# haowenz/FEM

Measured on AMD Instinct MI355X. Metric: mapped Mreads/s (100 bp, e=3) at 1/2/4/8 MI355X + achieved HBM GB/s vs roofline, higher is better.
Workload: dtype u32/u64 integer + 32-bit Myers bit-vectors

## Files before the change

fem_amd/csrc/fem_hip.hip:

```cpp
#include "../../include/fem_hip.h"

#include <hip/hip_runtime.h>
#include <rccl/rccl.h>
#include <sched.h>
#if defined(__x86_64__)
#include <immintrin.h>
#endif

#include <algorithm>
#include <cctype>
#include <cstdio>
#include <cstdlib>
#include <cstring>
#include <condition_variable>
#include <functional>
#include <atomic>
#include <chrono>
#include <mutex>
#include <string>
#include <thread>
#include <vector>

#include "fem_index_build.hip.h"
#include "fem_pack.h"
#include "fem_kernels.hip.h"
#include "fem_seed_fast.hip.h"
#include "fem_seed_join.hip.h"
#include "fem_tail.hip.h"
#include "fem_bgzf.hip.h"

namespace {

#ifndef FEM_SLOTS
#define FEM_SLOTS 4
#endif
constexpr int kSlots = FEM_SLOTS;
constexpr uint32_t kMaxReadLen = 1024;
constexpr size_t kFrontPad = 16;
constexpr uint32_t kXcapSmall = 512, kFcap = 128, kCcap = 128;

constexpr int kTimedKernels = 15;
struct TimedLaunch {
  int kernel;
  hipEvent_t start, stop;
  bool counts = true;
};
constexpr int kMaxParts = 4;

struct Slot {
  hipStream_t stream = nullptr;
  uint8_t *d_bases_alloc = nullptr;
  uint8_t *bases() const { return d_bases_alloc + 16; }
  size_t bases_cap = 0;
  uint64_t *d_off = nullptr;
  size_t off_cap = 0;
  uint64_t n_reads = 0;
  uint64_t n_bases = 0;
  uint32_t max_len = 0;
  bool staged = false;
  char *h_bases = nullptr;
  size_t h_bases_cap = 0;
  uint64_t *h_off = nullptr;
  size_t h_off_cap = 0;
  uint64_t acq_reads = 0, acq_bases = 0;
  char *h_quals = nullptr, *h_names = nullptr;
  uint64_t *h_name_off = nullptr;
  size_t h_quals_cap = 0, h_names_cap = 0, h_name_off_cap = 0;
  uint8_t *d_quals = nullptr, *d_names = nullptr;
  uint64_t *d_name_off = nullptr;
  size_t d_quals_cap = 0, d_names_cap = 0, d_name_off_cap = 0;
  bool text_staged = false;
  bool host_quals = false;
  const uint64_t *qual_at = nullptr;
  hipStream_t text_stream = nullptr;
  hipStream_t out_stream = nullptr;
  hipEvent_t ev_text_staged = nullptr;
  hipEvent_t ev_text_order = nullptr;
  bool have_text_order = false;
  uint8_t *d_packed = nullptr;
  size_t packed_cap = 0;
  uint32_t *d_exc_bits = nullptr;
  size_t exc_bits_cap = 0;
  uint32_t packed_bpr = 0;
  bool prefetch_results = false, staged_by_copy = false;
  uint64_t prefetched_reads2 = 0, prefetched_cand = 0, last_n_cand = 0;
  uint64_t h2d_bytes = 0;
  bool sent_packed = false;
  int parts = 1;
  uint32_t part_begin[kMaxParts + 1] = {0, 0, 0, 0, 0};
  hipEvent_t ev_part[kMaxParts] = {nullptr, nullptr, nullptr, nullptr}, ev_sel[kMaxParts] = {nullptr, nullptr, nullptr, nullptr};
  hipEvent_t ev_zeroed = nullptr;
  hipEvent_t ev_results = nullptr, ev_home = nullptr;
  uint64_t *d_cand = nullptr;
  uint32_t *d_meta = nullptr;
  uint8_t *d_ed = nullptr;
  int16_t *d_end = nullptr;
  uint32_t cand_cap = 0;
  uint32_t *d_begin = nullptr, *d_count = nullptr, *d_nmap = nullptr;
  size_t per_read_cap = 0;
  uint8_t *d_ctl = nullptr;
  uint8_t *h_ctl = nullptr;
  uint64_t *d_arena = nullptr;
  uint64_t arena_cap = 0;
  uint32_t *d_slow = nullptr;
  uint32_t slow_cap = 0;
  uint2 *d_sel = nullptr, *d_sel_hdr = nullptr;
  size_t sel_cap = 0, sel_hdr_cap = 0;
  uint32_t *h_begin = nullptr, *h_count = nullptr;
  size_t h_per_read_cap = 0;
  uint64_t *h_cand = nullptr;
  uint8_t *h_ed = nullptr;
  int16_t *h_end = nullptr;
// ... 93 lines not shown
  std::condition_variable cv_, done_;
  std::vector<std::thread> threads_;
  const std::function<void(unsigned)> *work_ = nullptr;
  unsigned n_ = 0, pending_ = 0;
  uint64_t epoch_ = 0;
  bool stop_ = false;
};
}

struct fem_dev {
  femt::TextGate text_gate;
  femz::Bgzf *bgzf = nullptr;
  uint8_t *d_zin = nullptr;
  size_t d_zin_cap = 0;
  hipStream_t z_stream = nullptr;
  std::recursive_mutex mu;
  int device = 0;
  StagePool *stage_pool = nullptr;
  uint8_t *d_ref_names = nullptr;
  uint32_t *d_ref_name_off = nullptr;
  int n_cu = 256;
  std::string err;
  uint32_t *d_lookup = nullptr;
  uint64_t n_lookup = 0;
  uint64_t *d_occ = nullptr;
  uint64_t n_occ = 0;
  int32_t k = 0, step = 0;
  uint64_t fast_occ_key = ~0ull;
  int fast_occ_blocks = 0;
  uint32_t *d_summary = nullptr;
  uint32_t *d_occ32 = nullptr, *d_goff = nullptr, *d_blkseq = nullptr;
  uint32_t list_shift = 0;
  bool no_strided = false;
  uint32_t *d_freq11 = nullptr;
  uint32_t n_banks = 1, bank_first[5] = {0, 0, 0, 0, 0};
  uint32_t *d_bank_lo = nullptr;
  uint64_t bank_limit = 0;
  uint32_t bank_seqs = 0;
  int select_occ_blocks = 0, join_occ_blocks = 0;
  uint64_t select_occ_key = ~0ull, join_occ_key = ~0ull;
  uint8_t *d_planes = nullptr;
  uint8_t *d_ref_raw = nullptr;
  uint64_t ref_bytes = 0;
  uint64_t *d_seq_off = nullptr;
  uint32_t *d_seq_len = nullptr;
  uint32_t n_seq = 0;
  std::vector<uint64_t> seq_off;
  std::vector<uint32_t> seq_len;
  Slot slot[kSlots];
  bool timing = false;
  int verify_blocks_per_cu = 0;
  double t_ms[kTimedKernels] = {};
  uint64_t t_n[kTimedKernels] = {};
  bool force_generic = false;
  bool force_hash = false;
  bool force_dense = false;
  bool no_dense = false;
  bool tiny_buffers = false;
  std::vector<hipEvent_t> event_pool;
  hipEvent_t ev_kernels_done = nullptr;
  bool have_kernels_done = false;
  hipEvent_t ev_select_done = nullptr;
  bool have_select_done = false;
  bool no_overlap = false;
  hipEvent_t ev_h2d_done = nullptr;
  bool have_h2d_done = false;
  hipStream_t side_stream = nullptr;
  bool no_parts = false;
  int max_parts = 2;
  bool timeline = false, have_epoch = false;
  hipEvent_t ev_epoch = nullptr;
};

namespace {

bool testing_switch(const char *name) {
  const char *t = getenv("FEM_TESTING");
  if (!(t && t[0] == '1')) return false;
  const char *v = getenv(name);
  return v && v[0] == '1';
}

int fail(fem_dev *h, int rc, const std::string &msg) {
  if (h) {
// ... 547 lines not shown
    *wpb_out = wpb, *lds_out = lds_bytes;
    *grid_out = (uint32_t)std::max<uint64_t>(1, std::min<uint64_t>(blocks_wanted, blocks_resident * 4));
  };
  if (sp.lay.wave_bytes > 64u * 1024u) return fail(h, FEM_ERR_UNSUPPORTED, "read too long for the device path");

  auto timed = [&](int id, hipStream_t st, auto &&launch, bool counts = true) -> int {
    TimedLaunch t{id, nullptr, nullptr, counts};
    if (h->timing) {
      t.start = get_event(h), t.stop = get_event(h);
      HIP_TRY(h, hipEventRecord(t.start, st));
    }
    launch();
    HIP_TRY(h, hipGetLastError());
    if (h->timing) {
      HIP_TRY(h, hipEventRecord(t.stop, st));
      s.pending.push_back(t);
    }
    return FEM_OK;
  };

  if (s.n_reads) {
    int rc;
    const bool split_dense = use_fast && h->d_occ32 && h->d_freq11;
    const bool overlap = split_dense && !h->no_overlap;
    if (!overlap && h->have_kernels_done) HIP_TRY(h, hipStreamWaitEvent(s.stream, h->ev_kernels_done, 0));
    femk::VerifyParams vp{};
    vp.bases = s.bases(), vp.read_off = s.d_off;
    vp.planes = h->d_planes, vp.seq_off = h->d_seq_off;
    vp.cand = s.d_cand, vp.cand_meta = s.d_meta;
    vp.ctr = d_ctr, vp.cand_cap = s.cand_cap, vp.e = p.e;
    vp.ed = s.d_ed, vp.end = s.d_end;
    vp.n_map = s.d_nmap, vp.stats = d_stats;
    HIP_TRY(h, hipMemsetAsync(s.d_nmap, 0, (size_t)s.n_reads * sizeof(uint32_t), s.stream));
    if (h->verify_blocks_per_cu == 0) {
      int nb = 0;
      if (hipOccupancyMaxActiveBlocksPerMultiprocessor(&nb, femk::verify_kernel, 256, 0) != hipSuccess || nb <= 0) nb = 4;
      h->verify_blocks_per_cu = nb;
    }
    const uint32_t vgrid = (uint32_t)h->n_cu * (uint32_t)h->verify_blocks_per_cu;
    if (split_dense) {
      const uint32_t max_len = std::max<uint32_t>(s.max_len, (uint32_t)p.k);
      const bool banked = h->n_banks > 1;
      const size_t want_sel = (size_t)s.n_reads * 6u * (size_t)R * h->n_banks;
      if ((rc = dev_realloc(h, &s.d_sel, &s.sel_cap, want_sel))) return rc;
      if ((rc = dev_realloc(h, &s.d_sel_hdr, &s.sel_hdr_cap, (size_t)s.n_reads))) return rc;
      femk::SeedParams fp = sp;
      fp.occ32 = h->d_occ32, fp.list_shift = h->list_shift, fp.goff = h->d_goff, fp.blkseq = h->d_blkseq;
      fp.freq11 = h->d_freq11, fp.sel = s.d_sel, fp.sel_hdr = s.d_sel_hdr;
      fp.n_banks = h->n_banks, fp.bank_lo = h->d_bank_lo, fp.n_buckets = (uint32_t)(h->n_lookup - 1);
      fp.blk_stride = (femk::kDenseRemap >> femk::kDenseBlkShift) + 1u;
      for (uint32_t b = 0; b <= femk::kDenseMaxBanks; ++b) fp.bank_first[b] = h->bank_first[b];
      uint32_t select_lds = 0, select_threads = 256;
      fp.lay = make_layout_select(p, max_len);
      if (fp.lay.wave_bytes > 64u * 1024u) return fail(h, FEM_ERR_UNSUPPORTED, "read too long for the device path");
      const femk::SeedLayout lay_select = fp.lay;
      femk::SeedLayout lay_join = make_layout_join(p, banked, !banked && h->list_shift != 0);
      const uint32_t wpb_s = std::min<uint32_t>(4u, std::max<uint32_t>(1u, (64u * 1024u) / lay_select.wave_bytes));
      const uint32_t wpb_j = std::min<uint32_t>(4u, std::max<uint32_t>(1u, (60u * 1024u) / lay_join.wave_bytes));
      lay_join.picked = wpb_j * lay_join.wave_bytes;
      const uint32_t lds_j = wpb_j * lay_join.wave_bytes + 64u * 8u;
      const int which = banked ? 1 : h->list_shift ? 2 : 0;
      uint64_t per_cu_s, per_cu_j;
      {
        const uint32_t lds_bytes = wpb_s * lay_select.wave_bytes;
        const uint64_t key = ((uint64_t)banked << 48) | ((uint64_t)R << 40) | lds_bytes;
        if (h->select_occ_key != key) h->select_occ_key = key, h->select_occ_blocks = select_blocks_per_cu(R, banked, (int)(64u * wpb_s), lds_bytes);
        per_cu_s = h->select_occ_blocks > 0 ? (uint64_t)h->select_occ_blocks : std::max<uint64_t>(1, 160u * 1024u / lds_bytes);
        if (overlap) per_cu_s = 1;
        select_lds = lds_bytes, select_threads = 64u * wpb_s;
      }
      {
        const uint64_t key = ((uint64_t)which << 48) | ((uint64_t)R << 40) | lds_j;
// ... 56 lines not shown
        if (h->fast_occ_key != key) h->fast_occ_key = key, h->fast_occ_blocks = fast_blocks_per_cu((int)R, hash, (int)(64u * wpb), lds_bytes);
        static const uint64_t mult = testing_switch("FEM_TESTING") && getenv("FEM_GRID_MULT") ? (uint64_t)std::max(1, atoi(getenv("FEM_GRID_MULT"))) : 1;
        const uint64_t per_cu = h->fast_occ_blocks > 0 ? (uint64_t)h->fast_occ_blocks : std::max<uint64_t>(1, 160u * 1024u / lds_bytes);
        const uint64_t wanted = (s.n_reads + (uint64_t)femk::kReadBlock * wpb - 1) / ((uint64_t)femk::kReadBlock * wpb);
        grid = (uint32_t)std::max<uint64_t>(1, std::min<uint64_t>(wanted, (uint64_t)h->n_cu * per_cu * mult));
      }
      auto launch_range = [&](uint32_t lo, uint32_t hi) {
        femk::SeedParams q = fp;
        q.read_begin = lo, q.n_reads = hi;
        dim3 g(grid), b(64u * wpb);
        switch (R) {
          case 1: launch_fast<1>(hash, g, b, lds_bytes, s.stream, q); break;
          case 2: launch_fast<2>(hash, g, b, lds_bytes, s.stream, q); break;
          case 3: launch_fast<3>(hash, g, b, lds_bytes, s.stream, q); break;
          case 4: launch_fast<4>(hash, g, b, lds_bytes, s.stream, q); break;
          case 5: launch_fast<5>(hash, g, b, lds_bytes, s.stream, q); break;
          case 6: launch_fast<6>(hash, g, b, lds_bytes, s.stream, q); break;
          case 7: launch_fast<7>(hash, g, b, lds_bytes, s.stream, q); break;
          case 8: launch_fast<8>(hash, g, b, lds_bytes, s.stream, q); break;
          case 9: launch_fast<9>(hash, g, b, lds_bytes, s.stream, q); break;
          default: launch_fast<10>(hash, g, b, lds_bytes, s.stream, q); break;
        }
      };
      rc = timed(0, s.stream, [&] { launch_range(0, (uint32_t)s.n_reads); });
      if (rc) return rc;
      sp.work_queue = s.d_slow;
    }
    {
      uint32_t wpb, lds_bytes, grid;
      shape(sp.lay, &wpb, &lds_bytes, &grid);
      rc = timed(2, s.stream, [&] { hipLaunchKernelGGL(femk::seed_filter_kernel, dim3(grid), dim3(64u * wpb), lds_bytes, s.stream, sp); });
      if (rc) return rc;
    }
    rc = timed(1, s.stream, [&] { hipLaunchKernelGGL(femk::verify_kernel, dim3(vgrid), dim3(256), 0, s.stream, vp); });
    if (rc) return rc;
    s.packed_enqueued = false, s.packed_home = 0, s.packed_per_read_home = false;
    if (s.want_packed && split_dense && (rc = enqueue_pack(h, s, true, false))) return rc;
    HIP_TRY(h, hipEventRecord(h->ev_kernels_done, s.stream));
    h->have_kernels_done = true;
    if (s.want_packed && (rc = enqueue_pack(h, s, !split_dense, true))) return rc;
  } else {
    s.packed_enqueued = false, s.packed_home = 0, s.packed_per_read_home = false;
  }
  HIP_TRY(h, hipMemcpyAsync(s.h_ctl, s.d_ctl, kCtlBytes, hipMemcpyDeviceToHost, s.stream));
  s.prefetched_reads2 = 0, s.prefetched_cand = 0;
  static const bool no_prefetch = testing_switch("FEM_NO_PREFETCH");
  if (s.prefetch_results && !s.want_packed && s.staged_by_copy && !no_prefetch) {
    hipStream_t st = d2h_begin(h, s);
    {
      Span span(h, s, 21, st);
      const size_t n2 = (size_t)s.n_reads * 2;
      if (n2 && s.h_begin && n2 <= s.h_per_read_cap) {
        HIP_TRY(h, hipMemcpyAsync(s.h_begin, s.d_begin, n2 * sizeof(uint32_t), hipMemcpyDeviceToHost, st));
        HIP_TRY(h, hipMemcpyAsync(s.h_count, s.d_count, n2 * sizeof(uint32_t), hipMemcpyDeviceToHost, st));
        s.prefetched_reads2 = n2;
      }
      const size_t guess = std::min<size_t>({(size_t)(s.last_n_cand + s.last_n_cand / 32 + 1024), s.h_cand_cap, (size_t)s.cand_cap});
      if (s.last_n_cand && s.h_cand && guess) {
        HIP_TRY(h, hipMemcpyAsync(s.h_cand, s.d_cand, guess * sizeof(uint64_t), hipMemcpyDeviceToHost, st));
        HIP_TRY(h, hipMemcpyAsync(s.h_ed, s.d_ed, guess * sizeof(uint8_t), hipMemcpyDeviceToHost, st));
        HIP_TRY(h, hipMemcpyAsync(s.h_end, s.d_end, guess * sizeof(int16_t), hipMemcpyDeviceToHost, st));
        s.prefetched_cand = guess;
      }
    }
    int rc2 = d2h_end(h, s, st);
    if (rc2) return rc2;
  }
// ... 126 lines not shown

struct CommSet {
  std::vector<int> devs;
  std::vector<ncclComm_t> comms;
  std::vector<uint64_t *> bufs;
};
std::mutex g_comm_mu;
CommSet *g_comm = nullptr;
void destroy_comm_set() {
  if (!g_comm) return;
  for (size_t i = 0; i < g_comm->devs.size(); ++i) {
    (void)hipSetDevice(g_comm->devs[i]);
    if (g_comm->bufs[i]) (void)hipFree(g_comm->bufs[i]);
    if (g_comm->comms[i]) ncclCommDestroy(g_comm->comms[i]);
  }
  delete g_comm;
  g_comm = nullptr;
}

int check_slot(fem_dev *h, int slot) {
  if (!h) return FEM_ERR_INVALID;
  if (slot < 0 || slot >= kSlots) return fail(h, FEM_ERR_INVALID, "slot out of range");
  return FEM_OK;
}


using fempack::pack_bases;

int enqueue_packed(fem_dev *h, Slot &s, uint64_t n, uint32_t len, uint64_t n_exc) {
  const uint32_t bpr = fempack::bytes_per_read(len);
  const uint64_t code_bytes = fempack::code_bytes(n, len), n_bases = n * (uint64_t)len;
  const uint64_t total = code_bytes + n_exc * 5u;
  int rc;
  if ((rc = dev_realloc(h, &s.d_packed, &s.packed_cap, (size_t)total + 64))) return rc;
  if ((rc = dev_realloc(h, &s.d_bases_alloc, &s.bases_cap, kFrontPad + (size_t)n_bases + 64))) return rc;
  if ((rc = dev_realloc(h, &s.d_off, &s.off_cap, (size_t)n + 1))) return rc;
  if ((rc = dev_realloc(h, &s.d_exc_bits, &s.exc_bits_cap, (size_t)n / 32 + 2))) return rc;
  s.parts = 1;
  if (!h->no_parts && !h->no_overlap && n_exc == 0 && n >= 2 * kPartMinReads && device_idle(h))
    s.parts = (int)std::min<uint64_t>((uint64_t)h->max_parts, n / kPartMinReads);
  for (int q = 0; q <= s.parts; ++q) s.part_begin[q] = q == s.parts ? (uint32_t)n : (uint32_t)((n * q / s.parts) & ~63ull);
  HIP_TRY(h, hipMemsetAsync(s.d_exc_bits, 0, ((size_t)n / 32 + 1) * sizeof(uint32_t), s.stream));
  hipLaunchKernelGGL(femk::uniform_offsets_kernel, dim3((uint32_t)std::min<uint64_t>((n + 256) / 256, (uint64_t)h->n_cu * 8u)), dim3(256), 0,
                     s.stream, s.d_off, n, len);
  if ((rc = h2d_begin(h, s))) return rc;
  for (int q = 0; q < s.parts; ++q) {
    const uint64_t r0 = s.part_begin[q], r1 = s.part_begin[q + 1];
    const uint64_t b0 = r0 * bpr, b1 = q + 1 == s.parts ? total : r1 * bpr;
    Span span(h, s, 20, s.stream);
    if (b1 > b0) HIP_TRY(h, hipMemcpyAsync(s.d_packed + b0, s.h_bases + b0, b1 - b0, hipMemcpyHostToDevice, s.stream));
    if (q + 1 == s.parts && (rc = h2d_end(h, s))) return rc;
    if (r1 > r0) {
      const uint32_t grid = (uint32_t)std::min<uint64_t>(((r1 - r0) * bpr + 255) / 256, (uint64_t)h->n_cu * 16u);
      hipLaunchKernelGGL(femk::unpack_reads_kernel, dim3(grid), dim3(256), 0, s.stream, (const uint8_t *)s.d_packed + b0, r1 - r0, len, bpr,
                         s.bases() + r0 * len);
    }
    if (s.parts > 1) HIP_TRY(h, hipEventRecord(s.ev_part[q], s.stream));
  }
  if (n_exc) {
    const dim3 g((uint32_t)std::min<uint64_t>((n_exc + 255) / 256, (uint64_t)h->n_cu * 4u));
    hipLaunchKernelGGL(femk::scatter_chars_kernel, g, dim3(256), 0, s.stream, (const uint32_t *)(s.d_packed + code_bytes),
                       (const uint8_t *)(s.d_packed + code_bytes + 4u * n_exc), n_exc, s.bases());
    hipLaunchKernelGGL(femk::mark_exception_reads_kernel, g, dim3(256), 0, s.stream, (const uint32_t *)(s.d_packed + code_bytes), n_exc, len,
                       s.d_exc_bits);
  }
  s.packed_bpr = bpr;
  HIP_TRY(h, hipGetLastError());
  s.n_reads = n, s.n_bases = n_bases, s.max_len = len;
  s.staged = true, s.mapped = false, s.synced = false;
  s.h2d_bytes = total, s.sent_packed = true;
  return FEM_OK;
}

unsigned stage_threads(uint64_t n_reads) {
  unsigned want = 12;
  if (const char *e = getenv("FEM_STAGE_THREADS")) want = (unsigned)std::max(1, atoi(e));
  const unsigned hw = std::thread::hardware_concurrency();
  return (unsigned)std::max<uint64_t>(1, std::min<uint64_t>({(uint64_t)(hw ? hw : 1), (uint64_t)want, n_reads / 65536 + 1}));
}

}

extern "C" {

const char *fem_strerror(int rc) {
  switch (rc) {
    case FEM_OK: return "ok";
    case FEM_ERR_INVALID: return "invalid argument";
    case FEM_ERR_HIP: return "HIP runtime error";
    case FEM_ERR_NOMEM: return "out of memory";
    case FEM_ERR_STATE: return "call order violated";
    case FEM_ERR_UNSUPPORTED: return "input not supported by the device path";
    case FEM_ERR_RCCL: return "RCCL error";
    default: return "unknown error";
  }
}
// ... 27 lines not shown
      delete h;
      return FEM_ERR_HIP;
    }
  }
  bool ok_ev = hipEventCreateWithFlags(&h->ev_kernels_done, hipEventDisableTiming) == hipSuccess &&
               hipEventCreateWithFlags(&h->ev_select_done, hipEventDisableTiming) == hipSuccess &&
               hipEventCreateWithFlags(&h->ev_h2d_done, hipEventDisableTiming) == hipSuccess &&
               hipStreamCreateWithFlags(&h->side_stream, hipStreamNonBlocking) == hipSuccess;
  for (int i = 0; ok_ev && i < kSlots; ++i) {
    Slot &sl = h->slot[i];
    ok_ev = hipEventCreateWithFlags(&sl.ev_zeroed, hipEventDisableTiming) == hipSuccess &&
            hipEventCreateWithFlags(&sl.ev_results, hipEventDisableTiming) == hipSuccess &&
            hipEventCreateWithFlags(&sl.ev_home, hipEventDisableTiming) == hipSuccess;
    for (int q = 0; ok_ev && q < kMaxParts; ++q)
      ok_ev = hipEventCreateWithFlags(&sl.ev_part[q], hipEventDisableTiming) == hipSuccess &&
              hipEventCreateWithFlags(&sl.ev_sel[q], hipEventDisableTiming) == hipSuccess;
  }
  if (!ok_ev) {
    (void)fem_dev_close(h);
    return FEM_ERR_HIP;
  }
  if (testing_switch("FEM_TESTING")) {
    h->no_overlap = testing_switch("FEM_NO_OVERLAP");
    h->no_parts = testing_switch("FEM_NO_PARTS");
    if (const char *mp = getenv("FEM_PARTS")) h->max_parts = std::min(kMaxParts, std::max(1, atoi(mp)));
    h->timeline = testing_switch("FEM_TIMELINE");
    if (h->timeline && hipEventCreate(&h->ev_epoch) == hipSuccess && hipEventRecord(h->ev_epoch, h->side_stream) == hipSuccess)
      h->timing = true, h->have_epoch = true;
    h->force_generic = testing_switch("FEM_FORCE_GENERIC");
    h->force_hash = testing_switch("FEM_FORCE_HASH");
    h->force_dense = testing_switch("FEM_FORCE_DENSE");
    h->no_dense = testing_switch("FEM_NO_DENSE");
    h->no_strided = testing_switch("FEM_NO_STRIDED");
    h->tiny_buffers = testing_switch("FEM_TEST_TINY_BUFFERS");
    if (const char *bl = getenv("FEM_TEST_BANK_BASES")) h->bank_limit = strtoull(bl, nullptr, 10);
    if (const char *bs = getenv("FEM_TEST_BANK_SEQS")) h->bank_seqs = (uint32_t)strtoul(bs, nullptr, 10);
  }
  *out = h;
  return FEM_OK;
}

int fem_dev_close(fem_dev *h) {
  if (!h) return FEM_ERR_INVALID;
  {
    std::lock_guard<std::mutex> lock(g_comm_mu);
    if (g_comm && std::find(g_comm->devs.begin(), g_comm->devs.end(), h->device) != g_comm->devs.end()) destroy_comm_set();
  }
  (void)hipSetDevice(h->device);
  (void)hipDeviceSynchronize();
  delete h->stage_pool;
  h->stage_pool = nullptr;
  for (auto &s : h->slot) {
    drain_timing(h, s);
    for (void *p : {(void *)s.d_bases_alloc, (void *)s.d_off, (void *)s.d_cand, (void *)s.d_meta, (void *)s.d_ed,
                    (void *)s.d_end, (void *)s.d_begin, (void *)s.d_count, (void *)s.d_nmap, (void *)s.d_ctl,
                    (void *)s.d_arena, (void *)s.d_slow, (void *)s.d_sel, (void *)s.d_sel_hdr, (void *)s.d_packed, (void *)s.d_exc_bits, (void *)s.d_quals, (void *)s.d_names,
                    (void *)s.d_name_off, (void *)s.d_count8, (void *)s.d_seg, (void *)s.d_pcand, (void *)s.d_ped, (void *)s.d_pend, (void *)s.d_big})
      if (p) (void)hipFree(p);
    for (void *p : {(void *)s.h_ctl, (void *)s.h_begin, (void *)s.h_count, (void *)s.h_cand, (void *)s.h_ed,
                    (void *)s.h_end, (void *)s.h_bases, (void *)s.h_off, (void *)s.h_quals, (void *)s.h_names, (void *)s.h_name_off,
                    (void *)s.h_count8, (void *)s.h_seg, (void *)s.h_pcand, (void *)s.h_ped, (void *)s.h_pend, (void *)s.h_big})
      if (p) (void)hipHostFree(p);
    if (s.stream) (void)hipStreamDestroy(s.stream);
    if (s.text_stream) (void)hipStreamDestroy(s.text_stream);
    if (s.out_stream) (void)hipStreamDestroy(s.out_stream);
    if (s.ev_text_staged) (void)hipEventDestroy(s.ev_text_staged);
    if (s.ev_text_order) (void)hipEventDestroy(s.ev_text_order);
    delete s.tail;
    s.tail = nullptr;
  }
  delete h->bgzf;
  h->bgzf = nullptr;
  if (h->d_zin) (void)hipFree(h->d_zin);
  if (h->z_stream) (void)hipStreamDestroy(h->z_stream);
  if (h->d_ref_names) (void)hipFree(h->d_ref_names);
  if (h->d_ref_name_off) (void)hipFree(h->d_ref_name_off);
  for (hipEvent_t e : h->event_pool) (void)hipEventDestroy(e);
  if (h->ev_kernels_done) (void)hipEventDestroy(h->ev_kernels_done);
  if (h->ev_select_done) (void)hipEventDestroy(h->ev_select_done);
  if (h->ev_h2d_done) (void)hipEventDestroy(h->ev_h2d_done);
  if (h->ev_epoch) (void)hipEventDestroy(h->ev_epoch);
  if (h->side_stream) (void)hipStreamDestroy(h->side_stream);
  for (int i = 0; i < kSlots; ++i) {
    Slot &sl = h->slot[i];
    if (sl.ev_zeroed) (void)hipEventDestroy(sl.ev_zeroed);
    if (sl.ev_results) (void)hipEventDestroy(sl.ev_results);
    if (sl.ev_home) (void)hipEventDestroy(sl.ev_home);
    for (int q = 0; q < kMaxParts; ++q) {
      if (sl.ev_part[q]) (void)hipEventDestroy(sl.ev_part[q]);
// ... 594 lines not shown
  return FEM_OK;
}

static hipStream_t out_stream_of(fem_dev *h, Slot &s) {
  static const bool plain = testing_switch("FEM_NO_OUT_PRIORITY");
  if (plain) return s.stream;
  if (!s.out_stream) {
    int least = 0, greatest = 0;
    if (hipDeviceGetStreamPriorityRange(&least, &greatest) != hipSuccess ||
        hipStreamCreateWithPriority(&s.out_stream, hipStreamNonBlocking, greatest) != hipSuccess)
      s.out_stream = nullptr;
  }
  (void)h;
  return s.out_stream ? s.out_stream : s.stream;
}

int fem_dev_reserve_batch(fem_dev *h, int slot, uint64_t n_reads, uint64_t n_records, uint32_t max_len, const fem_params *p) {
  int rc = check_slot(h, slot);
  if (rc) return rc;
  FEM_LOCK(h);
  if (!params_ok(p)) return fail(h, FEM_ERR_INVALID, "parameters out of range (k 1..16, step 1..16, e 0..7, a 0..2)");
  if (!h->d_lookup) return fail(h, FEM_ERR_STATE, "the index must be uploaded first (what a batch needs depends on it)");
  if (n_reads == 0 || n_reads > 0x7FFFFFF0ull || n_records > 0xFFFFFFF0ull || max_len == 0 || max_len > kMaxReadLen)
    return fail(h, FEM_ERR_INVALID, "batch shape out of range");
  Slot &s = h->slot[slot];
  if (s.mapped && !s.synced) return fail(h, FEM_ERR_STATE, "a batch is in flight in this slot");
  HIP_TRY(h, hipSetDevice(h->device));
  const uint64_t n_was = s.n_reads;
  s.n_reads = n_reads;
  rc = ensure_outputs(h, s);
  s.n_reads = n_was;
  if (rc) return rc;
  const uint64_t n_bases = n_reads * (uint64_t)max_len;
  if ((rc = dev_realloc(h, &s.d_packed, &s.packed_cap, (size_t)fempack::code_bytes(n_reads, max_len) + 64))) return rc;
  if ((rc = dev_realloc(h, &s.d_bases_alloc, &s.bases_cap, kFrontPad + (size_t)n_bases + 64))) return rc;
  if ((rc = dev_realloc(h, &s.d_off, &s.off_cap, (size_t)n_reads + 1))) return rc;
  if ((rc = dev_realloc(h, &s.d_exc_bits, &s.exc_bits_cap, (size_t)n_reads / 32 + 2))) return rc;
  if (h->d_occ32 && h->d_freq11 && p->k == 12 && p->step == 3) {
    const size_t R = (size_t)(p->e + 1 + p->a);
    if ((rc = dev_realloc(h, &s.d_sel, &s.sel_cap, (size_t)n_reads * 6u * R * h->n_banks))) return rc;
    if ((rc = dev_realloc(h, &s.d_sel_hdr, &s.sel_hdr_cap, (size_t)n_reads))) return rc;
  }
  if (!s.tail) s.tail = new (std::nothrow) femt::Tail();
  if (!s.tail) return fail(h, FEM_ERR_NOMEM, "out of host memory");
  std::string err;
  if ((rc = s.tail->reserve((uint32_t)n_reads, (uint32_t)n_records, max_len, p->e, h->tiny_buffers, &err))) return fail(h, rc, err);
  if (!s.text_stream) HIP_TRY(h, hipStreamCreateWithFlags(&s.text_stream, hipStreamNonBlocking));
  HIP_TRY(h, hipMemsetAsync(s.d_sel_hdr ? (void *)s.d_sel_hdr : (void *)s.d_off, 0, 8, s.text_stream));
  HIP_TRY(h, hipStreamSynchronize(s.text_stream));
  HIP_TRY(h, hipMemsetAsync(s.d_off, 0, 8, h->side_stream));
  HIP_TRY(h, hipStreamSynchronize(h->side_stream));
  const size_t probe = 1u << 20;
  if (s.h_bases && s.h_bases_cap >= probe && s.bases_cap >= kFrontPad + probe)
    HIP_TRY(h, hipMemcpyAsync(s.d_bases_alloc + kFrontPad, s.h_bases, probe, hipMemcpyHostToDevice, s.stream));
  if (s.h_quals && s.d_quals && s.h_quals_cap >= probe && s.d_quals_cap >= probe)
    HIP_TRY(h, hipMemcpyAsync(s.d_quals, s.h_quals, probe, hipMemcpyHostToDevice, s.text_stream));
  HIP_TRY(h, hipMemcpyAsync(s.h_ctl, s.d_ctl, kCtlBytes, hipMemcpyDeviceToHost, s.stream));
  HIP_TRY(h, hipStreamSynchronize(s.text_stream));
  HIP_TRY(h, hipStreamSynchronize(s.stream));
  if ((rc = s.tail->warm(out_stream_of(h, s), &err))) return fail(h, rc, err);
  return FEM_OK;
}

static int commit_text(fem_dev *h, int slot, uint64_t n_reads, uint64_t n_name_bytes, bool with_quals) {
  int rc = check_slot(h, slot);
  if (rc) return rc;
  FEM_LOCK(h);
// ... 31 lines not shown
  if (!qual_at) return fail(h, FEM_ERR_INVALID, "null output pointer");
  if (!s.host_quals || !s.qual_at) return fail(h, FEM_ERR_STATE, "the slot's last SAM text was rendered with its qualities (or there is none)");
  *qual_at = s.qual_at;
  if (n_reads) *n_reads = s.n_reads;
  return FEM_OK;
}

static int fetch_sam(fem_dev *h, int slot, fem_batch_sam *out, bool wait);
int fem_dev_fetch_sam(fem_dev *h, int slot, fem_batch_sam *out) { return fetch_sam(h, slot, out, true); }
int fem_dev_fetch_sam_nowait(fem_dev *h, int slot, fem_batch_sam *out) { return fetch_sam(h, slot, out, false); }
int fem_dev_sam_wait(fem_dev *h, int slot) {
  if (!h || slot < 0 || slot >= kSlots) return FEM_ERR_INVALID;
  Slot &s = h->slot[slot];
  if (!s.tail) return FEM_ERR_STATE;
  if (hipSetDevice(h->device) != hipSuccess) return FEM_ERR_HIP;
  return s.tail->wait_text();
}

static int rescue_input(fem_dev *h, const Slot &s, femt::RescueInput *ri) {
  if (!s.rescue) return FEM_OK;
  if ((int64_t)s.max_insert - s.min_insert > 65536)
    return fail(h, FEM_ERR_UNSUPPORTED, "mate rescue searches insert windows of at most 65536 (max_insert - min_insert)");
  ri->max_edits = s.rescue_edits;
  ri->bases = s.bases(), ri->read_off = s.d_off, ri->max_len = s.max_len;
  ri->ref_raw = h->d_ref_raw, ri->ref_bytes = h->ref_bytes + 64, ri->seq_off = h->d_seq_off, ri->seq_len = h->d_seq_len;
  return FEM_OK;
}

static femt::TailInput tail_input(const fem_dev *h, const Slot &s) {
  femt::TailInput in{};
  in.bases = s.bases(), in.read_off = s.d_off, in.n_reads = (uint32_t)s.n_reads, in.max_len = s.max_len;
  in.ref_raw = h->d_ref_raw, in.ref_bytes = h->ref_bytes + 64, in.seq_off = h->d_seq_off;
  in.planes = h->d_planes;
  if (s.sent_packed) in.packed = s.d_packed, in.packed_bpr = s.packed_bpr, in.exc_bits = s.d_exc_bits;
  in.cand = s.d_cand, in.ed = s.d_ed, in.end = s.d_end, in.cand_begin = s.d_begin, in.cand_count = s.d_count;
  in.n_map = s.d_nmap, in.e = s.params.e, in.n_records = s.stats[4];
  return in;
}

struct TailFront {
  femt::TailInput in;
  femt::TailOutput t;
  hipStream_t stream;
  double ms[3], ms_sync, ms_run;
  std::chrono::steady_clock::time_point t_in;
};

static int tail_records(fem_dev *h, int slot, const void *out, bool copy_records, bool device_quals, TailFront *f) {
  f->t_in = std::chrono::steady_clock::now();
  auto since = [&]() { return std::chrono::duration<double, std::milli>(std::chrono::steady_clock::now() - f->t_in).count(); };
  int rc = fem_dev_sync(h, slot);
  if (rc) return rc;
  f->ms_sync = since();
  if (!out) return fail(h, FEM_ERR_INVALID, "null result");
  Slot &s = h->slot[slot];
  const bool text = !copy_records, paired = text && s.paired;
  if (text && !s.text_staged) return fail(h, FEM_ERR_STATE, "qualities and names of this batch were not committed (fem_dev_commit_text_stage)");
  if (device_quals && s.host_quals) return fail(h, FEM_ERR_STATE, "BAM records need the qualities on the device (fem_dev_commit_text_stage, not _names_stage)");
  if (text && !h->d_ref_names) return fail(h, FEM_ERR_STATE, "reference names must be uploaded first (fem_dev_upload_reference_names)");
  s.prefetch_results = false;
  if (!s.tail) s.tail = new (std::nothrow) femt::Tail();
  if (!s.tail) return fail(h, FEM_ERR_NOMEM, "out of host memory");
  f->in = tail_input(h, s);
  if (paired && (s.n_reads & 1)) return fail(h, FEM_ERR_INVALID, "a batch of read pairs holds an even number of reads");
  if (copy_records && s.out_stream) HIP_TRY(h, hipStreamSynchronize(s.out_stream));
  f->stream = copy_records ? s.stream : out_stream_of(h, s);
  std::string err;
// ... 493 lines not shown
```

fem_amd/csrc/fem_kernels.hip.h:

```cpp
#pragma once
#include <hip/hip_runtime.h>
#include <stdint.h>
#include "fem_planes.hip.h"

namespace femk {

constexpr int kWave = 64;
constexpr uint32_t kFlagCandOverflow = 1u;
constexpr uint32_t kFlagArenaOverflow = 2u;
constexpr uint32_t kFlagTooLarge = 4u;
constexpr uint32_t kInvalidMeta = 0xFFFFFFFFu;
constexpr int kMaxR = 10;
constexpr uint32_t kMeta16 = 0x80000000u;
constexpr uint32_t kSlotChunk = 256u;
constexpr uint32_t kFlagQueueOverflow = 8u;
constexpr uint32_t kQueueChunk = 32u;
constexpr uint32_t kInvalidRead = 0xFFFFFFFFu;

struct SeedLayout {
  uint32_t pkw, nkw;
  uint32_t sf;
  uint32_t dp_rows;
  uint32_t dp_bits;
  uint32_t picked;
// ... 1102 lines not shown
          } else {
            if (ln == 0) atomicOr(&p.ctr[1], kFlagTooLarge);
          }
        }
      }
      wave_sync_lds();
      STAMP(prof, 7);
    }
  }
  pad_chunk(p, chunk);
#ifdef FEM_STAMPS
  prof.flush();
#endif
  if (ln == 0) {
    if (pre_sum) atomicAdd(&p.stats[0], pre_sum);
    if (cand_sum) atomicAdd(&p.stats[1], cand_sum);
  }
}

struct VerifyParams {
  const uint8_t *bases;
  const uint64_t *read_off;
  const uint8_t *planes;
  const uint64_t *seq_off;
  const uint64_t *cand;
  const uint32_t *cand_meta;
  const uint32_t *ctr;
  uint32_t cand_cap;
  int32_t e;
  uint8_t *ed;
  int16_t *end;
  uint32_t *n_map;
  unsigned long long *stats;
};

__device__ __forceinline__ uint4 load_u128_unaligned(const uint8_t *p) {
  uint4 w;
  __builtin_memcpy(&w, p, 16);
  return w;
}

__device__ __forceinline__ uint4 plane_window(const uint8_t *planes, int q, uint64_t at) {
  return load_u128_unaligned(plane_addr(planes, q, at));
}
__device__ __forceinline__ uint32_t load_u32_unaligned(const uint8_t *p) {
  uint32_t w;
  __builtin_memcpy(&w, p, 4);
  return w;
}

struct MyersState {
  uint32_t VP, VN;
  int score;
};

__device__ __forceinline__ void decode4(uint32_t chars, uint32_t complement, uint32_t &code, uint32_t &nflag) {
  const uint32_t t = (chars >> 1) & 0x03030303u;
  const uint32_t c = t ^ ((t >> 1) & 0x01010101u);
  const uint32_t upper = chars & 0xDFDFDFDFu;
  const uint32_t expect = __builtin_amdgcn_perm(0u, 0x54474341u , c);
  const uint32_t z = upper ^ expect;
  nflag = ((((z & 0x7F7F7F7Fu) + 0x7F7F7F7Fu) | z) >> 7) & 0x01010101u;
  code = (c ^ complement) & ~(nflag * 3u);
}

__device__ __forceinline__ uint32_t window_head(const uint4 &w, uint32_t off) { return __builtin_amdgcn_alignbit(w.y, w.x, off); }
// ... 99 lines not shown
      }
      rejected = m.score > 3 * e;
    }
    int score = m.score;
    int best = score, endp = L - 1;
    if (!rejected) {
      for (int j = 0; j < 2 * e; ++j) {
        score += (int)((m.VP >> j) & 1u) - (int)((m.VN >> j) & 1u);
        if (score < best) {
          best = score;
          endp = L + j;
        }
      }
    }
    const bool accepted = !rejected && best <= e;
    p.ed[i] = accepted ? (uint8_t)best : (uint8_t)0xFF;
    p.end[i] = accepted ? (int16_t)endp : (int16_t)0;
    {
      const uint32_t ln = lane_id();
      const uint64_t acc = __ballot(accepted);
      const uint32_t prev_read = __shfl_up(read, 1);
      const bool joins_prev = accepted && ln > 0u && ((acc >> (ln - 1u)) & 1ull) && prev_read == read;
      const uint64_t heads = __ballot(accepted && !joins_prev);
      if (accepted && !joins_prev) {
        const uint64_t stop = (heads | ~acc) >> ln >> 1;
        const uint32_t run = stop ? (uint32_t)__builtin_ctzll(stop) + 1u : 64u - ln;
        mapped += (uint32_t)(atomicAdd(&p.n_map[read], run) == 0u);
      }
      if (accepted) ++mappings;
    }
  }
  for (int d = 32; d >= 1; d >>= 1) mappings += __shfl_xor(mappings, d), mapped += __shfl_xor(mapped, d);
  __syncthreads();
  if (lane_id() == 0) part[0][threadIdx.x >> 6] = mappings, part[1][threadIdx.x >> 6] = mapped;
  __syncthreads();
  if (threadIdx.x == 0) {
    const uint32_t a = part[0][0] + part[0][1] + part[0][2] + part[0][3], b = part[1][0] + part[1][1] + part[1][2] + part[1][3];
    if (a) atomicAdd(&p.stats[2], (unsigned long long)a);
    if (b) atomicAdd(&p.stats[3], (unsigned long long)b);
  }
}

struct PackParams {
  const uint32_t *cand_begin, *cand_count;
  const uint64_t *cand;
  const uint8_t *ed;
  const int16_t *end;
  const uint32_t *ctr;
  uint32_t n_strands;
  uint8_t *count8;
  uint32_t *seg_begin;
  uint64_t *pcand;
  uint8_t *ped;
  int16_t *pend;
  uint32_t pcap;
  uint32_t *cursor;
  uint2 *big;
  uint32_t big_cap;
};
constexpr uint32_t kPackSegs = 16;
__global__ void __launch_bounds__(256) pack_results_kernel(PackParams p) {
  if (p.ctr[1] != 0) return;
  __shared__ uint32_t part[kPackSegs * 4u];
  __shared__ uint32_t block_base;
  const uint32_t seg0 = blockIdx.x * kPackSegs;
  const uint32_t wave = threadIdx.x >> 6;
// ... 98 lines not shown
```

Baseline: 374.0.

## Verify candidates directly from 2-bit packed reads instead of unpacked chars

Adds a verify kernel variant that reads the 2-bit packed read codes, loading 64 bases per 16-byte text load and reverse-complementing via bit tricks. Reads flagged as containing exception characters fall back to the char path. This cuts read-text bandwidth and decode work in the Myers verification loop, at the cost of extra branching, a per-candidate exception-bit load, and a front pad on the packed buffer so the reverse-strand address arithmetic stays in bounds. The new path is taken whenever packed reads were sent, unless the FEM_VERIFY_CHARS switch is set.

```diff
diff --git a/fem_amd/csrc/fem_hip.hip b/fem_amd/csrc/fem_hip.hip
--- a/fem_amd/csrc/fem_hip.hip
+++ b/fem_amd/csrc/fem_hip.hip
@@ -37,6 +37,7 @@
 constexpr int kSlots = FEM_SLOTS;
 constexpr uint32_t kMaxReadLen = 1024;
 constexpr size_t kFrontPad = 16;
+constexpr size_t kPackedFrontPad = 256;
 constexpr uint32_t kXcapSmall = 512, kFcap = 128, kCcap = 128;
 
 constexpr int kTimedKernels = 15;
@@ -77,7 +78,8 @@
   hipEvent_t ev_text_staged = nullptr;
   hipEvent_t ev_text_order = nullptr;
   bool have_text_order = false;
-  uint8_t *d_packed = nullptr;
+  uint8_t *d_packed_alloc = nullptr;
+  uint8_t *packed() const { return d_packed_alloc + kPackedFrontPad; }
   size_t packed_cap = 0;
   uint32_t *d_exc_bits = nullptr;
   size_t exc_bits_cap = 0;
@@ -237,6 +239,7 @@
   uint32_t *d_occ32 = nullptr, *d_goff = nullptr, *d_blkseq = nullptr;
   uint32_t list_shift = 0;
   bool no_strided = false;
+  bool verify_chars = false;
   uint32_t *d_freq11 = nullptr;
   uint32_t n_banks = 1, bank_first[5] = {0, 0, 0, 0, 0};
   uint32_t *d_bank_lo = nullptr;
@@ -255,6 +258,7 @@
   Slot slot[kSlots];
   bool timing = false;
   int verify_blocks_per_cu = 0;
+  int verify_packed_blocks_per_cu = 0;
   double t_ms[kTimedKernels] = {};
   uint64_t t_n[kTimedKernels] = {};
   bool force_generic = false;
@@ -868,12 +872,17 @@
     vp.ed = s.d_ed, vp.end = s.d_end;
     vp.n_map = s.d_nmap, vp.stats = d_stats;
     HIP_TRY(h, hipMemsetAsync(s.d_nmap, 0, (size_t)s.n_reads * sizeof(uint32_t), s.stream));
-    if (h->verify_blocks_per_cu == 0) {
+    const bool verify_packed = s.sent_packed && !h->verify_chars;
+    if (verify_packed) vp.packed = s.packed(), vp.exc_bits = s.d_exc_bits, vp.bpr = s.packed_bpr, vp.len = s.max_len;
+    int &v_per_cu = verify_packed ? h->verify_packed_blocks_per_cu : h->verify_blocks_per_cu;
+    if (v_per_cu == 0) {
       int nb = 0;
-      if (hipOccupancyMaxActiveBlocksPerMultiprocessor(&nb, femk::verify_kernel, 256, 0) != hipSuccess || nb <= 0) nb = 4;
-      h->verify_blocks_per_cu = nb;
-    }
-    const uint32_t vgrid = (uint32_t)h->n_cu * (uint32_t)h->verify_blocks_per_cu;
+      const hipError_t qe = verify_packed ? hipOccupancyMaxActiveBlocksPerMultiprocessor(&nb, femk::verify_kernel_packed, 256, 0)
+                                          : hipOccupancyMaxActiveBlocksPerMultiprocessor(&nb, femk::verify_kernel, 256, 0);
+      if (qe != hipSuccess || nb <= 0) nb = 4;
+      v_per_cu = nb;
+    }
+    const uint32_t vgrid = (uint32_t)h->n_cu * (uint32_t)v_per_cu;
     if (split_dense) {
       const uint32_t max_len = std::max<uint32_t>(s.max_len, (uint32_t)p.k);
       const bool banked = h->n_banks > 1;
@@ -996,7 +1005,10 @@
       rc = timed(2, s.stream, [&] { hipLaunchKernelGGL(femk::seed_filter_kernel, dim3(grid), dim3(64u * wpb), lds_bytes, s.stream, sp); });
       if (rc) return rc;
     }
-    rc = timed(1, s.stream, [&] { hipLaunchKernelGGL(femk::verify_kernel, dim3(vgrid), dim3(256), 0, s.stream, vp); });
+    rc = timed(1, s.stream, [&] {
+      if (verify_packed) hipLaunchKernelGGL(femk::verify_kernel_packed, dim3(vgrid), dim3(256), 0, s.stream, vp);
+      else hipLaunchKernelGGL(femk::verify_kernel, dim3(vgrid), dim3(256), 0, s.stream, vp);
+    });
     if (rc) return rc;
     s.packed_enqueued = false, s.packed_home = 0, s.packed_per_read_home = false;
     if (s.want_packed && split_dense && (rc = enqueue_pack(h, s, true, false))) return rc;
@@ -1189,7 +1201,7 @@
   const uint64_t code_bytes = fempack::code_bytes(n, len), n_bases = n * (uint64_t)len;
   const uint64_t total = code_bytes + n_exc * 5u;
   int rc;
-  if ((rc = dev_realloc(h, &s.d_packed, &s.packed_cap, (size_t)total + 64))) return rc;
+  if ((rc = dev_realloc(h, &s.d_packed_alloc, &s.packed_cap, kPackedFrontPad + (size_t)total + 64))) return rc;
   if ((rc = dev_realloc(h, &s.d_bases_alloc, &s.bases_cap, kFrontPad + (size_t)n_bases + 64))) return rc;
   if ((rc = dev_realloc(h, &s.d_off, &s.off_cap, (size_t)n + 1))) return rc;
   if ((rc = dev_realloc(h, &s.d_exc_bits, &s.exc_bits_cap, (size_t)n / 32 + 2))) return rc;
@@ -1205,20 +1217,20 @@
     const uint64_t r0 = s.part_begin[q], r1 = s.part_begin[q + 1];
     const uint64_t b0 = r0 * bpr, b1 = q + 1 == s.parts ? total : r1 * bpr;
     Span span(h, s, 20, s.stream);
-    if (b1 > b0) HIP_TRY(h, hipMemcpyAsync(s.d_packed + b0, s.h_bases + b0, b1 - b0, hipMemcpyHostToDevice, s.stream));
+    if (b1 > b0) HIP_TRY(h, hipMemcpyAsync(s.packed() + b0, s.h_bases + b0, b1 - b0, hipMemcpyHostToDevice, s.stream));
     if (q + 1 == s.parts && (rc = h2d_end(h, s))) return rc;
     if (r1 > r0) {
       const uint32_t grid = (uint32_t)std::min<uint64_t>(((r1 - r0) * bpr + 255) / 256, (uint64_t)h->n_cu * 16u);
-      hipLaunchKernelGGL(femk::unpack_reads_kernel, dim3(grid), dim3(256), 0, s.stream, (const uint8_t *)s.d_packed + b0, r1 - r0, len, bpr,
+      hipLaunchKernelGGL(femk::unpack_reads_kernel, dim3(grid), dim3(256), 0, s.stream, (const uint8_t *)s.packed() + b0, r1 - r0, len, bpr,
                          s.bases() + r0 * len);
     }
     if (s.parts > 1) HIP_TRY(h, hipEventRecord(s.ev_part[q], s.stream));
   }
   if (n_exc) {
     const dim3 g((uint32_t)std::min<uint64_t>((n_exc + 255) / 256, (uint64_t)h->n_cu * 4u));
-    hipLaunchKernelGGL(femk::scatter_chars_kernel, g, dim3(256), 0, s.stream, (const uint32_t *)(s.d_packed + code_bytes),
-                       (const uint8_t *)(s.d_packed + code_bytes + 4u * n_exc), n_exc, s.bases());
-    hipLaunchKernelGGL(femk::mark_exception_reads_kernel, g, dim3(256), 0, s.stream, (const uint32_t *)(s.d_packed + code_bytes), n_exc, len,
+    hipLaunchKernelGGL(femk::scatter_chars_kernel, g, dim3(256), 0, s.stream, (const uint32_t *)(s.packed() + code_bytes),
+                       (const uint8_t *)(s.packed() + code_bytes + 4u * n_exc), n_exc, s.bases());
+    hipLaunchKernelGGL(femk::mark_exception_reads_kernel, g, dim3(256), 0, s.stream, (const uint32_t *)(s.packed() + code_bytes), n_exc, len,
                        s.d_exc_bits);
   }
   s.packed_bpr = bpr;
@@ -1312,6 +1324,7 @@
     h->force_dense = testing_switch("FEM_FORCE_DENSE");
     h->no_dense = testing_switch("FEM_NO_DENSE");
     h->no_strided = testing_switch("FEM_NO_STRIDED");
+    h->verify_chars = testing_switch("FEM_VERIFY_CHARS");
     h->tiny_buffers = testing_switch("FEM_TEST_TINY_BUFFERS");
     if (const char *bl = getenv("FEM_TEST_BANK_BASES")) h->bank_limit = strtoull(bl, nullptr, 10);
     if (const char *bs = getenv("FEM_TEST_BANK_SEQS")) h->bank_seqs = (uint32_t)strtoul(bs, nullptr, 10);
@@ -1334,7 +1347,7 @@
     drain_timing(h, s);
     for (void *p : {(void *)s.d_bases_alloc, (void *)s.d_off, (void *)s.d_cand, (void *)s.d_meta, (void *)s.d_ed,
                     (void *)s.d_end, (void *)s.d_begin, (void *)s.d_count, (void *)s.d_nmap, (void *)s.d_ctl,
-                    (void *)s.d_arena, (void *)s.d_slow, (void *)s.d_sel, (void *)s.d_sel_hdr, (void *)s.d_packed, (void *)s.d_exc_bits, (void *)s.d_quals, (void *)s.d_names,
+                    (void *)s.d_arena, (void *)s.d_slow, (void *)s.d_sel, (void *)s.d_sel_hdr, (void *)s.d_packed_alloc, (void *)s.d_exc_bits, (void *)s.d_quals, (void *)s.d_names,
                     (void *)s.d_name_off, (void *)s.d_count8, (void *)s.d_seg, (void *)s.d_pcand, (void *)s.d_ped, (void *)s.d_pend, (void *)s.d_big})
       if (p) (void)hipFree(p);
     for (void *p : {(void *)s.h_ctl, (void *)s.h_begin, (void *)s.h_count, (void *)s.h_cand, (void *)s.h_ed,
@@ -1995,7 +2008,7 @@
   s.n_reads = n_was;
   if (rc) return rc;
   const uint64_t n_bases = n_reads * (uint64_t)max_len;
-  if ((rc = dev_realloc(h, &s.d_packed, &s.packed_cap, (size_t)fempack::code_bytes(n_reads, max_len) + 64))) return rc;
+  if ((rc = dev_realloc(h, &s.d_packed_alloc, &s.packed_cap, kPackedFrontPad + (size_t)fempack::code_bytes(n_reads, max_len) + 64))) return rc;
   if ((rc = dev_realloc(h, &s.d_bases_alloc, &s.bases_cap, kFrontPad + (size_t)n_bases + 64))) return rc;
   if ((rc = dev_realloc(h, &s.d_off, &s.off_cap, (size_t)n_reads + 1))) return rc;
   if ((rc = dev_realloc(h, &s.d_exc_bits, &s.exc_bits_cap, (size_t)n_reads / 32 + 2))) return rc;
@@ -2093,7 +2106,7 @@
   in.bases = s.bases(), in.read_off = s.d_off, in.n_reads = (uint32_t)s.n_reads, in.max_len = s.max_len;
   in.ref_raw = h->d_ref_raw, in.ref_bytes = h->ref_bytes + 64, in.seq_off = h->d_seq_off;
   in.planes = h->d_planes;
-  if (s.sent_packed) in.packed = s.d_packed, in.packed_bpr = s.packed_bpr, in.exc_bits = s.d_exc_bits;
+  if (s.sent_packed) in.packed = s.packed(), in.packed_bpr = s.packed_bpr, in.exc_bits = s.d_exc_bits;
   in.cand = s.d_cand, in.ed = s.d_ed, in.end = s.d_end, in.cand_begin = s.d_begin, in.cand_count = s.d_count;
   in.n_map = s.d_nmap, in.e = s.params.e, in.n_records = s.stats[4];
   return in;
diff --git a/fem_amd/csrc/fem_kernels.hip.h b/fem_amd/csrc/fem_kernels.hip.h
--- a/fem_amd/csrc/fem_kernels.hip.h
+++ b/fem_amd/csrc/fem_kernels.hip.h
@@ -1158,6 +1158,9 @@
   int16_t *end;
   uint32_t *n_map;
   unsigned long long *stats;
+  const uint8_t *packed;
+  const uint32_t *exc_bits;
+  uint32_t bpr, len;
 };
 
 __device__ __forceinline__ uint4 load_u128_unaligned(const uint8_t *p) {
@@ -1323,6 +1326,194 @@
   }
   for (int d = 32; d >= 1; d >>= 1) mappings += __shfl_xor(mappings, d), mapped += __shfl_xor(mapped, d);
   __syncthreads();
+  if (lane_id() == 0) part[0][threadIdx.x >> 6] = mappings, part[1][threadIdx.x >> 6] = mapped;
+  __syncthreads();
+  if (threadIdx.x == 0) {
+    const uint32_t a = part[0][0] + part[0][1] + part[0][2] + part[0][3], b = part[1][0] + part[1][1] + part[1][2] + part[1][3];
+    if (a) atomicAdd(&p.stats[2], (unsigned long long)a);
+    if (b) atomicAdd(&p.stats[3], (unsigned long long)b);
+  }
+}
+
+__device__ __forceinline__ uint32_t reverse_fields2(uint32_t x) {
+  x = __builtin_bitreverse32(x);
+  return ((x >> 1) & 0x55555555u) | ((x & 0x55555555u) << 1);
+}
+
+constexpr int kStepsPerTextLoad = 4;
+
+__device__ __forceinline__ bool verify_walk_packed(const VerifyParams &p, MyersState &m, const uint8_t *row, uint32_t strand, uint64_t pat,
+                                                   int L, int e, uint32_t width, uint32_t wm) {
+  const int n_steps = (L + 15) >> 4;
+  bool rejected = false;
+  const uint32_t sh = strand ? 2u * ((uint32_t)L & 3u) : 0u;
+  auto text_addr = [&](int col) { return strand == 0 ? row + (col >> 2) : row + ((L - 64 - col) >> 2); };
+  auto plane_chunk = [&](int q, int col) { return plane_window(p.planes, q, (pat + (uint32_t)col) >> 3); };
+  uint4 P0 = make_uint4(0, 0, 0, 0), P1 = P0, P2 = P0, P0n = P0, P1n = P0, P2n = P0, T = P0, Tn = P0;
+  uint32_t Tn4 = 0;
+  if (n_steps > 0) {
+    const uint8_t *a = text_addr(0);
+    Tn = load_u128_unaligned(a);
+    if (sh) Tn4 = load_u32_unaligned(a + 16);
+    P0n = plane_chunk(0, 0), P1n = plane_chunk(1, 0), P2n = plane_chunk(2, 0);
+  }
+  const uint32_t pat_bit = (uint32_t)pat & 7u;
+  for (int step = 0; step < n_steps && !rejected; ++step) {
+    const int col = step << 4, sub = step % kStepsPerPlaneLoad;
+    if (step % kStepsPerTextLoad == 0) {
+      T = Tn;
+      const uint32_t t4 = Tn4;
+      if (step + kStepsPerTextLoad < n_steps) {
+        const uint8_t *a = text_addr(col + 16 * kStepsPerTextLoad);
+        Tn = load_u128_unaligned(a);
+        if (sh) Tn4 = load_u32_unaligned(a + 16);
+      }
+      if (strand) {
+        const uint32_t a0 = __builtin_amdgcn_alignbit(T.y, T.x, sh), a1 = __builtin_amdgcn_alignbit(T.z, T.y, sh);
+        const uint32_t a2 = __builtin_amdgcn_alignbit(T.w, T.z, sh), a3 = __builtin_amdgcn_alignbit(t4, T.w, sh);
+        T = make_uint4(~reverse_fields2(a3), ~reverse_fields2(a2), ~reverse_fields2(a1), ~reverse_fields2(a0));
+      }
+    } else {
+      T.x = T.y, T.y = T.z, T.z = T.w;
+    }
+    if (sub == 0) {
+      P0 = P0n, P1 = P1n, P2 = P2n;
+      if (step + kStepsPerPlaneLoad < n_steps) {
+        const int nc = col + 16 * kStepsPerPlaneLoad;
+        P0n = plane_chunk(0, nc), P1n = plane_chunk(1, nc), P2n = plane_chunk(2, nc);
+      }
+    } else {
+      window_advance16(P0), window_advance16(P1), window_advance16(P2);
+    }
+    const uint32_t b0 = window_head(P0, pat_bit), b1 = window_head(P1, pat_bit), b2 = window_head(P2, pat_bit);
+    const uint32_t t = T.x;
+    if (col + 16 <= L) {
+#pragma unroll
+      for (int q = 0; q < 16; ++q) {
+        const uint32_t m0 = (uint32_t)__builtin_amdgcn_sbfe((int)t, 2 * q, 1);
+        const uint32_t m1 = (uint32_t)__builtin_amdgcn_sbfe((int)t, 2 * q + 1, 1);
+        myers_column(m, b0, b1, b2, m0, m1, 0u, (uint32_t)q, width, wm);
+      }
+    } else {
+      for (int q = 0; q < L - col; ++q) {
+        const uint32_t cb = t >> (2 * q);
+        myers_column(m, b0, b1, b2, 0u - (cb & 1u), 0u - ((cb >> 1) & 1u), 0u, (uint32_t)q, width, wm);
+      }
+    }
+    rejected = m.score > 3 * e;
+  }
+  return rejected;
+}
+
+__device__ __forceinline__ bool verify_walk_chars(const VerifyParams &p, MyersState &m, const uint8_t *rd, uint32_t strand, uint64_t pat,
+                                                  int L, int e, uint32_t width, uint32_t wm) {
+  const int n_steps = (L + 15) >> 4;
+  bool rejected = false;
+  const uint32_t complement = strand ? 0x03030303u : 0u;
+  const uint32_t pat_bit = (uint32_t)pat & 7u;
+  uint4 P0 = make_uint4(0, 0, 0, 0), P1 = P0, P2 = P0;
+  for (int step = 0; step < n_steps && !rejected; ++step) {
+    const int col = step << 4;
+    if (step % kStepsPerPlaneLoad == 0) {
+      const uint64_t at = (pat + (uint32_t)col) >> 3;
+      P0 = plane_window(p.planes, 0, at), P1 = plane_window(p.planes, 1, at), P2 = plane_window(p.planes, 2, at);
+    } else {
+      window_advance16(P0), window_advance16(P1), window_advance16(P2);
+    }
+    const uint4 r = load_u128_unaligned(strand == 0 ? rd + col : rd + (L - 16 - col));
+    const uint32_t b0 = window_head(P0, pat_bit), b1 = window_head(P1, pat_bit), b2 = window_head(P2, pat_bit);
+    uint32_t cw[4], nw[4];
+    decode4(strand ? __builtin_bswap32(r.w) : r.x, complement, cw[0], nw[0]);
+    decode4(strand ? __builtin_bswap32(r.z) : r.y, complement, cw[1], nw[1]);
+    decode4(strand ? __builtin_bswap32(r.y) : r.z, complement, cw[2], nw[2]);
+    decode4(strand ? __builtin_bswap32(r.x) : r.w, complement, cw[3], nw[3]);
+    const uint64_t clo = ((uint64_t)cw[1] << 32) | cw[0], chi = ((uint64_t)cw[3] << 32) | cw[2];
+    const uint64_t nlo = ((uint64_t)nw[1] << 32) | nw[0], nhi = ((uint64_t)nw[3] << 32) | nw[2];
+    const int n_col = L - col < 16 ? L - col : 16;
+    for (int q = 0; q < n_col; ++q) {
+      const uint32_t cb = (uint32_t)((q < 8 ? clo : chi) >> (8 * (q & 7)));
+      const uint32_t nb = (uint32_t)((q < 8 ? nlo : nhi) >> (8 * (q & 7)));
+      myers_column(m, b0, b1, b2, 0u - (cb & 1u), 0u - ((cb >> 1) & 1u), 0u - (nb & 1u), (uint32_t)q, width, wm);
+    }
+    rejected = m.score > 3 * e;
+  }
+  return rejected;
+}
+
+__global__ void __launch_bounds__(256, 6) verify_kernel_packed(VerifyParams p) {
+  if (p.ctr[1] != 0) return;
+  const uint32_t total = min(p.ctr[0], p.cand_cap);
+  const uint32_t stride = gridDim.x * blockDim.x;
+  const int e = p.e, L = (int)p.len;
+  const uint32_t width = 2u * (uint32_t)e + 1u;
+  __shared__ uint32_t part[2][4];
+  uint32_t mappings = 0, mapped = 0;
+  uint32_t i = blockIdx.x * blockDim.x + threadIdx.x;
+  uint32_t meta_n = kInvalidMeta, exc_n = 0;
+  uint64_t c_n = 0, seq_off_n = 0;
+  auto request_second = [&] {
+    if (meta_n != kInvalidMeta) {
+      seq_off_n = p.seq_off[(uint32_t)(c_n >> 32)];
+      exc_n = p.exc_bits[(meta_n & ~kMeta16) >> 6];
+    }
+  };
+  if (i < total) {
+    meta_n = p.cand_meta[i], c_n = p.cand[i];
+    request_second();
+  }
+  while (i < total) {
+    const uint32_t meta = meta_n, exc_word = exc_n;
+    const uint64_t c = c_n, seq_off = seq_off_n;
+    const uint32_t at = i;
+    const uint32_t next = i + stride;
+    i = next > at ? next : total;
+    meta_n = kInvalidMeta;
+    if (i < total) meta_n = p.cand_meta[i], c_n = p.cand[i];
+    if (meta == kInvalidMeta) {
+      p.ed[at] = 0xFF, p.end[at] = 0;
+      request_second();
+      continue;
+    }
+    const uint32_t read = (meta & ~kMeta16) >> 1, strand = meta & 1u;
+    const uint32_t wm = (meta & kMeta16) ? 0xFFFFu : 0xFFFFFFFFu;
+    const uint64_t pat = seq_off + (uint32_t)c;
+    MyersState m{0, 0, 0};
+    bool rejected;
+    if ((exc_word >> (read & 31u)) & 1u) {
+      rejected = verify_walk_chars(p, m, p.bases + (uint64_t)read * (uint32_t)L, strand, pat, L, e, width, wm);
+    } else {
+      rejected = verify_walk_packed(p, m, p.packed + (uint64_t)read * p.bpr, strand, pat, L, e, width, wm);
+    }
+    request_second();
+    int score = m.score;
+    int best = score, endp = L - 1;
+    if (!rejected) {
+      for (int j = 0; j < 2 * e; ++j) {
+        score += (int)((m.VP >> j) & 1u) - (int)((m.VN >> j) & 1u);
+        if (score < best) {
+          best = score;
+          endp = L + j;
+        }
+      }
+    }
+    const bool accepted = !rejected && best <= e;
+    p.ed[at] = accepted ? (uint8_t)best : (uint8_t)0xFF;
+    p.end[at] = accepted ? (int16_t)endp : (int16_t)0;
+    {
+      const uint32_t ln = lane_id();
+      const uint64_t acc = __ballot(accepted);
+      const uint32_t prev_read = __shfl_up(read, 1);
+      const bool joins_prev = accepted && ln > 0u && ((acc >> (ln - 1u)) & 1ull) && prev_read == read;
+      const uint64_t heads = __ballot(accepted && !joins_prev);
+      if (accepted && !joins_prev) {
+        const uint64_t stop = (heads | ~acc) >> ln >> 1;
+        const uint32_t run = stop ? (uint32_t)__builtin_ctzll(stop) + 1u : 64u - ln;
+        mapped += (uint32_t)(atomicAdd(&p.n_map[read], run) == 0u);
+      }
+      if (accepted) ++mappings;
+    }
+  }
+  for (int d = 32; d >= 1; d >>= 1) mappings += __shfl_xor(mappings, d), mapped += __shfl_xor(mapped, d);
   if (lane_id() == 0) part[0][threadIdx.x >> 6] = mappings, part[1][threadIdx.x >> 6] = mapped;
   __syncthreads();
   if (threadIdx.x == 0) {
```

New measurement: 378.2, median of 6. 1.01x the previous value.
